# NTHU-LSALAB/KubeShare

Hardware: AMD Instinct MI355X
Metric: aggregate images/sec, co-located shared-GPU pods (higher is better)
Workload: dtype bf16; 1 GPU; model=resnet50, global_batch=512, image_size=224, parallelism=2 pods @ request=0.5, 2/GPU, pods_per_gpu=2, miopen_find=False, lease_accounting=sampled-busy

## Files before the change

kubeshare_amd/models/conv.py:

```python
import torch
import torch.nn as nn


class LowpConv2d(nn.Conv2d):
    _lowp_weight = None

    def _split_input(self, x, w):
        if self.bias is not None or self.padding_mode != "zeros" \
                or isinstance(self.padding, str):
            return None
        if not (w.is_cuda and x.is_cuda and w.dtype == torch.bfloat16
                and x.dim() == 4):
            return None
        from .. import ops
        if not ops.wrw_stream_enabled():
            return None
        if x.dtype != torch.bfloat16:
            if not (x.is_floating_point()
                    and torch.is_autocast_enabled("cuda")
                    and torch.get_autocast_dtype("cuda") == torch.bfloat16):
                return None
            x = x.to(torch.bfloat16)
        return x

    def forward(self, x):
        w = self._lowp_weight
        if w is None:
            return super().forward(x)
        xs = self._split_input(x, w)
        if xs is None:
            return self._conv_forward(x, w, self.bias)
        from .. import ops
        return ops.conv2d_split(xs, w, self.stride, self.padding,
                                self.dilation, self.groups)
```

kubeshare_amd/ops/__init__.py:

```python
from __future__ import annotations

import os

_HERE = os.path.dirname(os.path.abspath(__file__))
_BUILD_DIR = os.path.join(_HERE, "_build")
_SRCS = [os.path.join(_HERE, "hip", "ks_ops.hip"),
         os.path.join(_HERE, "hip", "bn_relu.hip"),
         os.path.join(_HERE, "hip", "pool.hip"),
         os.path.join(_HERE, "hip", "bn_pool.hip"),
         os.path.join(_HERE, "hip", "bn_join.hip"),
         os.path.join(_HERE, "hip", "bias_relu.hip"),
         os.path.join(_HERE, "hip", "cast.hip"),
         os.path.join(_HERE, "hip", "conv_split.hip"),
         os.path.join(_HERE, "hip", "grad_bucket.hip")]

_ext = None


def build_extension(verbose: bool = False):
    import torch
    from torch.utils import cpp_extension

    os.environ.setdefault("PYTORCH_ROCM_ARCH", "gfx950")
    os.makedirs(_BUILD_DIR, exist_ok=True)
# ... 322 lines not shown
                 and x.is_contiguous(memory_format=torch.channels_last))
    if supported and res is not None and res.dtype != torch.bfloat16:
        res = res.to(torch.bfloat16)
    if not supported:
        y = torch.nn.functional.batch_norm(
            x, bn.running_mean, bn.running_var, bn.weight, bn.bias,
            bn.training, bn.momentum, bn.eps)
        if res is not None:
            y = y + res
        y = torch.relu(y) if relu else y
        return (y, y) if fork else y
    if res is not None and not res.is_contiguous(
            memory_format=torch.channels_last):
        res = res.contiguous(memory_format=torch.channels_last)
    fn = _bn_relu_autograd()
    return fn.apply(x, res, bn.weight, bn.bias, bn.running_mean,
                    bn.running_var, bn.training, bn.momentum, bn.eps, relu,
                    fork)


_BNJoinFn = None


def bn_join_enabled() -> bool:
    return os.environ.get("KUBESHARE_BN_JOIN", "1") != "0"


def _bn_join_autograd():
    global _BNJoinFn
    if _BNJoinFn is not None:
        return _BNJoinFn
    import torch

    class BNJoinFn(torch.autograd.Function):

        @staticmethod
        def forward(ctx, x, x_d, weight, bias, running_mean, running_var,
                    momentum, eps, weight_d, bias_d, running_mean_d,
                    running_var_d, momentum_d, eps_d, fork):
            ext = _load()
            w32, b32 = weight.float(), bias.float()
            wd32, bd32 = weight_d.float(), bias_d.float()
            ctx.set_materialize_grads(False)
            ctx.wdtype = weight.dtype
            ctx.wdtype_d = weight_d.dtype
            ctx.legacy_reduce = bn_reduce_legacy()
            ctx.masked = bn_mask_enabled()
            out = ext.bn_join_fwd_train(
                x, w32, b32, running_mean, running_var, momentum, eps,
                x_d, wd32, bd32, running_mean_d, running_var_d, momentum_d,
                eps_d, ctx.masked, ctx.legacy_reduce)
            y = out[0]
            ctx.save_for_backward(x, x_d, out[5] if ctx.masked else y, w32,
                                  wd32, *out[1:5])
            return (y, y.view_as(y)) if fork else y

        @staticmethod
        def backward(ctx, dy, dy2=None):
            x, x_d, ym, w32, wd32, mean, invstd, mean_d, invstd_d = \
                ctx.saved_tensors
            if dy is None:
                dy, dy2 = dy2, None
            if dy is None:
                return (None,) * 15
            dx, dx_d, dscale, dbias, dscale_d = _load().bn_join_bwd(
                x, x_d, ym, dy, dy2, w32, wd32, mean, invstd, mean_d,
                invstd_d, ctx.masked, ctx.legacy_reduce)
            return (dx, dx_d, dscale.to(ctx.wdtype), dbias.to(ctx.wdtype),
                    None, None, None, None, dscale_d.to(ctx.wdtype_d),
                    dbias.clone().to(ctx.wdtype_d), None, None, None, None,
                    None)

    _BNJoinFn = BNJoinFn
    return BNJoinFn


def bn_join_supported(x, x_d) -> bool:
    import torch

    return (x.dim() == 4 and x.shape == x_d.shape
            and x.size(1) % 8 == 0 and x.size(1) <= 2048
            and all(t.is_cuda and t.dtype == torch.bfloat16
                    and t.is_contiguous(memory_format=torch.channels_last)
                    for t in (x, x_d)))


def bn_join(x, bn, x_d, bn_d, fork=False):
    if not (bn_join_enabled() and bn.training and bn_d.training
            and bn_join_supported(x, x_d)):
        return bn_relu(x, bn, res=bn_relu(x_d, bn_d, relu=False), fork=fork)
    fn = _BNJoinFn or _bn_join_autograd()
    return fn.apply(x, x_d, bn.weight, bn.bias, bn.running_mean,
                    bn.running_var, bn.momentum, bn.eps, bn_d.weight,
                    bn_d.bias, bn_d.running_mean, bn_d.running_var,
                    bn_d.momentum, bn_d.eps, fork)


_CastWeightsFn = None


def _cast_weights_autograd():
    global _CastWeightsFn
    if _CastWeightsFn is not None:
        return _CastWeightsFn
    import torch

    class CastWeightsFn(torch.autograd.Function):

        @staticmethod
        def forward(ctx, *weights):
            ctx.set_materialize_grads(False)
            return tuple(_load().cast_f32_to_bf16_multi(list(weights)))

        @staticmethod
        def backward(ctx, *grads):
            wgrad_join()
            out = list(grads)
            idx = [i for i, g in enumerate(grads)
                   if g is not None and g.dtype == torch.bfloat16]
            if idx:
                cast = _load().cast_bf16_to_f32_multi(
                    [grads[i] for i in idx])
                for i, g in zip(idx, cast):
                    out[i] = g
            return tuple(out)

    _CastWeightsFn = CastWeightsFn
    return CastWeightsFn


def cast_weights_bf16(weights):
    fn = _CastWeightsFn or _cast_weights_autograd()
    return fn.apply(*weights)


def lowp_weights_enabled() -> bool:
    return os.environ.get("KUBESHARE_LOWP_WEIGHTS", "1") != "0"


def stage_lowp_weights(convs):
    import torch

    if not convs or not lowp_weights_enabled():
        return []
    if not torch.is_autocast_enabled("cuda") or \
            torch.get_autocast_dtype("cuda") != torch.bfloat16:
        return []
    weights = [m.weight for m in convs]
    if not all(w.is_cuda and w.dtype == torch.float32 for w in weights):
        return []
    wgrad_join()
    for m, w in zip(convs, cast_weights_bf16(weights)):
        m._lowp_weight = w
    return convs


def clear_lowp_weights(convs):
    for m in convs:
        m._lowp_weight = None


def wrw_stream_enabled() -> bool:
    return os.environ.get("KUBESHARE_WRW_STREAM", "1") != "0"


def conv2d_split(x, w, stride=(1, 1), padding=(0, 0), dilation=(1, 1),
                 groups=1):
    def two(v):
        return [int(v), int(v)] if isinstance(v, int) else [int(i) for i in v]
    return _load().conv2d_split(x, w, two(stride), two(padding),
                                two(dilation), int(groups))


def wgrad_join():
    if _ext is not None:
        _ext.wgrad_join()


_POOL_CONFIGS = ((3, 2, 1), (2, 2, 0))
_MaxPoolNHWCFn = None


def _pool_int(v):
    if type(v) is int:
        return v
    if isinstance(v, (tuple, list)) and len(v) == 2 and v[0] == v[1] \
            and type(v[0]) is int:
        return v[0]
    return None


def _pool_cfg(kernel_size, stride, padding):
    if stride is None or stride == () or stride == []:
        stride = kernel_size
    return (_pool_int(kernel_size), _pool_int(stride), _pool_int(padding))


def _pool_cfg_supported(x, cfg) -> bool:
    import torch

    if cfg not in _POOL_CONFIGS or x.dim() != 4:
        return False
    n, c, h, w = x.shape
    k, _, p = cfg
    return (x.is_cuda and x.dtype == torch.bfloat16
            and c % 8 == 0 and 8 <= c <= 2048 and n >= 1
            and h + 2 * p >= k and w + 2 * p >= k
            and n * h * w < 2 ** 31
            and x.is_contiguous(memory_format=torch.channels_last))


def fused_pool_enabled() -> bool:
    return os.environ.get("KUBESHARE_FUSED_POOL", "1") != "0"


def max_pool_supported(x, kernel_size, stride=None, padding=0) -> bool:
    return _pool_cfg_supported(x, _pool_cfg(kernel_size, stride, padding))


def _max_pool_autograd():
    global _MaxPoolNHWCFn
    if _MaxPoolNHWCFn is not None:
        return _MaxPoolNHWCFn
    import torch
    from torch.autograd.function import once_differentiable

    class MaxPoolNHWCFn(torch.autograd.Function):

        @staticmethod
        def forward(ctx, x, k, s, p, want_idx):
            out = _load().max_pool_nhwc_fwd(x, k, s, p, want_idx)
            if want_idx:
                ctx.save_for_backward(out[1])
                ctx.input_sizes = list(x.shape)
                ctx.cfg = (k, s, p)
            return out[0]

        @staticmethod
        @once_differentiable
        def backward(ctx, dy):
            (idx,) = ctx.saved_tensors
            if not dy.is_contiguous(memory_format=torch.channels_last):
                dy = dy.contiguous(memory_format=torch.channels_last)
            k, s, p = ctx.cfg
            dx = _load().max_pool_nhwc_bwd(dy, idx, ctx.input_sizes,
                                           k, s, p)
            return dx, None, None, None, None

    _MaxPoolNHWCFn = MaxPoolNHWCFn
    return MaxPoolNHWCFn


def max_pool_nhwc(x, kernel_size, stride=None, padding=0):
    import torch

    cfg = _pool_cfg(kernel_size, stride, padding)
    if not _pool_cfg_supported(x, cfg):
        return torch.nn.functional.max_pool2d(x, kernel_size, stride,
                                              padding)
    want_idx = torch.is_grad_enabled() and x.requires_grad
    fn = _MaxPoolNHWCFn or _max_pool_autograd()
    return fn.apply(x, *cfg, want_idx)


_BNReLUMaxPoolNHWCFn = None


def bn_pool_enabled() -> bool:
    return os.environ.get("KUBESHARE_BN_POOL", "1") != "0"


def bn_relu_pool_supported(x, kernel_size, stride=None, padding=0) -> bool:
    return _pool_cfg_supported(x, _pool_cfg(kernel_size, stride, padding))


def _bn_relu_pool_autograd():
    global _BNReLUMaxPoolNHWCFn
    if _BNReLUMaxPoolNHWCFn is not None:
        return _BNReLUMaxPoolNHWCFn
    import torch
    from torch.autograd.function import once_differentiable

    class BNReLUMaxPoolNHWCFn(torch.autograd.Function):

        @staticmethod
        def forward(ctx, x, weight, bias, running_mean, running_var,
                    training, momentum, eps, k, s, p, want_idx):
            ext = _load()
            w32 = weight.float()
            b32 = bias.float()
            if not training:
                return ext.bn_relu_pool_fwd_eval(
                    x, w32, b32, running_mean.float(), running_var.float(),
                    eps, k, s, p)[0]
            legacy = bn_reduce_legacy()
            out = ext.bn_relu_pool_fwd_train(
                x, w32, b32, running_mean, running_var, momentum, eps,
                k, s, p, want_idx, legacy)
            if want_idx:
                ctx.save_for_backward(x, out[3], out[1], out[2], w32, b32)
                ctx.cfg = (k, s, p)
                ctx.wdtype = weight.dtype
                ctx.legacy_reduce = legacy
            return out[0]

        @staticmethod
        @once_differentiable
        def backward(ctx, dy):
            x, idx, mean, invstd, w32, b32 = ctx.saved_tensors
            if not dy.is_contiguous(memory_format=torch.channels_last):
                dy = dy.contiguous(memory_format=torch.channels_last)
            dx, dscale, dbias = _load().bn_relu_pool_bwd(
                x, dy, idx, w32, b32, mean, invstd, *ctx.cfg,
                ctx.legacy_reduce)
            return (dx, dscale.to(ctx.wdtype), dbias.to(ctx.wdtype)) + \
                (None,) * 9

    _BNReLUMaxPoolNHWCFn = BNReLUMaxPoolNHWCFn
    return BNReLUMaxPoolNHWCFn


def bn_relu_pool(x, bn, kernel_size, stride=None, padding=0):
    import torch

    cfg = _pool_cfg(kernel_size, stride, padding)
    fused = bn_pool_enabled() and _pool_cfg_supported(x, cfg)
    want_idx = False
    if fused:
        want_idx = torch.is_grad_enabled() and (
            x.requires_grad or bn.weight.requires_grad
            or bn.bias.requires_grad)
        fused = bn.training or not want_idx
    if not fused:
        return max_pool_nhwc(bn_relu(x, bn), kernel_size, stride, padding)
    fn = _BNReLUMaxPoolNHWCFn or _bn_relu_pool_autograd()
    return fn.apply(x, bn.weight, bn.bias, bn.running_mean, bn.running_var,
                    bn.training, bn.momentum, bn.eps, *cfg, want_idx)


_BiasReLUFn = None
_BiasReLUMaxPoolNHWCFn = None


def bias_relu_enabled() -> bool:
    return os.environ.get("KUBESHARE_BIAS_RELU", "1") != "0"


def bias_relu_supported(x) -> bool:
    import torch

    if x.dim() != 4:
        return False
    n, c, h, w = x.shape
    return (x.is_cuda and x.dtype == torch.bfloat16
            and c % 8 == 0 and 8 <= c <= 2048
            and n >= 1 and h >= 1 and w >= 1 and n * h * w < 2 ** 31
            and x.is_contiguous(memory_format=torch.channels_last))


def bias_relu_pool_supported(x, kernel_size, stride=None, padding=0) -> bool:
    return _pool_cfg_supported(x, _pool_cfg(kernel_size, stride, padding))


def _bias_relu_autograd():
    global _BiasReLUFn
    if _BiasReLUFn is not None:
        return _BiasReLUFn
    import torch
    from torch.autograd.function import once_differentiable

    class BiasReLUFn(torch.autograd.Function):

        @staticmethod
        def forward(ctx, x, bias):
            y = _load().bias_relu_fwd(
                x, bias.detach().float().contiguous())
            ctx.save_for_backward(y)
            ctx.bdtype = bias.dtype
            return y

        @staticmethod
        @once_differentiable
        def backward(ctx, dy):
            (y,) = ctx.saved_tensors
            if not dy.is_contiguous(memory_format=torch.channels_last):
                dy = dy.contiguous(memory_format=torch.channels_last)
            dx, db = _load().bias_relu_bwd(dy, y)
            return dx, db.to(ctx.bdtype)

    _BiasReLUFn = BiasReLUFn
    return BiasReLUFn


def _bias_relu_pool_autograd():
    global _BiasReLUMaxPoolNHWCFn
    if _BiasReLUMaxPoolNHWCFn is not None:
        return _BiasReLUMaxPoolNHWCFn
    import torch
    from torch.autograd.function import once_differentiable

    class BiasReLUMaxPoolNHWCFn(torch.autograd.Function):

        @staticmethod
        def forward(ctx, x, bias, k, s, p, want_idx):
            out = _load().bias_relu_pool_fwd(
                x, bias.detach().float().contiguous(), k, s, p, want_idx)
            if want_idx:
                ctx.save_for_backward(out[1], out[0])
                ctx.input_sizes = list(x.shape)
                ctx.cfg = (k, s, p)
                ctx.bdtype = bias.dtype
            return out[0]

        @staticmethod
        @once_differentiable
        def backward(ctx, dy):
            idx, y = ctx.saved_tensors
            if not dy.is_contiguous(memory_format=torch.channels_last):
                dy = dy.contiguous(memory_format=torch.channels_last)
            dx, db = _load().bias_relu_pool_bwd(dy, idx, y, ctx.input_sizes,
                                                *ctx.cfg)
            return dx, db.to(ctx.bdtype), None, None, None, None

    _BiasReLUMaxPoolNHWCFn = BiasReLUMaxPoolNHWCFn
    return BiasReLUMaxPoolNHWCFn


def bias_relu(x, bias):
    import torch

    if not bias_relu_supported(x) or not bias.is_cuda:
        return torch.relu(x + bias.to(x.dtype).view(1, -1, 1, 1))
    fn = _BiasReLUFn or _bias_relu_autograd()
    return fn.apply(x, bias)


def bias_relu_pool(x, bias, kernel_size, stride=None, padding=0):
    import torch

    cfg = _pool_cfg(kernel_size, stride, padding)
    if not _pool_cfg_supported(x, cfg) or not bias.is_cuda:
        if bias_relu_supported(x) and bias.is_cuda:
            return max_pool_nhwc(bias_relu(x, bias), kernel_size, stride,
                                 padding)
        y = torch.relu(x + bias.to(x.dtype).view(1, -1, 1, 1))
        return torch.nn.functional.max_pool2d(y, kernel_size, stride,
                                              padding)
    want_idx = torch.is_grad_enabled() and (x.requires_grad
                                            or bias.requires_grad)
    fn = _BiasReLUMaxPoolNHWCFn or _bias_relu_pool_autograd()
    return fn.apply(x, bias, *cfg, want_idx)


class PendingBNReLU:

    __slots__ = ("x", "bn")

    def __init__(self, x, bn):
        self.x = x
        self.bn = bn

    def materialize(self):
        return bn_relu(self.x, self.bn)


def fuse_model(model):
    _load()
    for m in model.modules():
        if hasattr(m, "fused_ops"):
            m.fused_ops = True
    return model
```

kubeshare_amd/ops/hip/cast.hip:

```cpp
#include <hip/hip_runtime.h>
#include <torch/extension.h>
#include <ATen/cuda/CUDAContext.h>

#include <vector>

#include "cast_common.h"

#define KS_CAST_THREADS 256
#define KS_CAST_VPT 4
#define KS_CAST_CHUNK (KS_CAST_THREADS * KS_CAST_VPT * 8)
#define KS_CAST_MAX_TENSORS 128

typedef __attribute__((ext_vector_type(8))) unsigned short cast_ushort8;

struct CastMultiArgs {
  const void* src[KS_CAST_MAX_TENSORS];
  void* dst[KS_CAST_MAX_TENSORS];
  long long n[KS_CAST_MAX_TENSORS];
  int blk[KS_CAST_MAX_TENSORS + 1];
  int count;
};
static_assert(sizeof(CastMultiArgs) <= 4096,
              "CastMultiArgs must fit the 4 KiB kernel-argument segment");

// ... 18 lines not shown
  CastF8 f;
  f.lo = make_float4(cast_bf16_to_f32(u[0]), cast_bf16_to_f32(u[1]),
                     cast_bf16_to_f32(u[2]), cast_bf16_to_f32(u[3]));
  f.hi = make_float4(cast_bf16_to_f32(u[4]), cast_bf16_to_f32(u[5]),
                     cast_bf16_to_f32(u[6]), cast_bf16_to_f32(u[7]));
  return f;
}

template <bool TO_BF16>
__global__ void __launch_bounds__(KS_CAST_THREADS)
cast_multi_kernel(const CastMultiArgs a) {
  const int b = blockIdx.x;
  int lo = 0, hi = a.count - 1;
  while (lo < hi) {
    int mid = (lo + hi + 1) >> 1;
    if (a.blk[mid] <= b) lo = mid; else hi = mid - 1;
  }
  const long long base = (long long)(b - a.blk[lo]) * KS_CAST_CHUNK;
  const long long rem = a.n[lo] - base;
  const int len = rem < KS_CAST_CHUNK ? (int)rem : KS_CAST_CHUNK;
  const float* __restrict__ f32p;
  const unsigned short* __restrict__ srcb;
  float* __restrict__ dstf;
  unsigned short* __restrict__ bf16p;
  if (TO_BF16) {
    f32p = static_cast<const float*>(a.src[lo]) + base;
    bf16p = static_cast<unsigned short*>(a.dst[lo]) + base;
  } else {
    srcb = static_cast<const unsigned short*>(a.src[lo]) + base;
    dstf = static_cast<float*>(a.dst[lo]) + base;
  }
  const int tid = threadIdx.x;
  const bool vec = TO_BF16
      ? (((uintptr_t)f32p | (uintptr_t)bf16p) & 15) == 0
      : (((uintptr_t)srcb | (uintptr_t)dstf) & 15) == 0;
  if (!vec) {
    for (int k = tid; k < len; k += KS_CAST_THREADS) {
      if (TO_BF16) bf16p[k] = cast_f32_to_bf16(f32p[k]);
      else dstf[k] = cast_bf16_to_f32(srcb[k]);
    }
    return;
  }
  const int len8 = len >> 3;
  if (TO_BF16) {
    const float4* s4 = reinterpret_cast<const float4*>(f32p);
    cast_ushort8* d8 = reinterpret_cast<cast_ushort8*>(bf16p);
    if (len == KS_CAST_CHUNK) {
      CastF8 v[KS_CAST_VPT];
#pragma unroll
      for (int u = 0; u < KS_CAST_VPT; u++) {
        const int k = tid + u * KS_CAST_THREADS;
        v[u].lo = s4[2 * k];
        v[u].hi = s4[2 * k + 1];
      }
#pragma unroll
      for (int u = 0; u < KS_CAST_VPT; u++)
        d8[tid + u * KS_CAST_THREADS] = cast_pack8(v[u]);
      return;
    }
    for (int k = tid; k < len8; k += KS_CAST_THREADS) {
      CastF8 v;
      v.lo = s4[2 * k];
      v.hi = s4[2 * k + 1];
      d8[k] = cast_pack8(v);
    }
    for (int k = len8 * 8 + tid; k < len; k += KS_CAST_THREADS)
      bf16p[k] = cast_f32_to_bf16(f32p[k]);
  } else {
    const cast_ushort8* s8 = reinterpret_cast<const cast_ushort8*>(srcb);
    float4* d4 = reinterpret_cast<float4*>(dstf);
    if (len == KS_CAST_CHUNK) {
      cast_ushort8 v[KS_CAST_VPT];
#pragma unroll
      for (int u = 0; u < KS_CAST_VPT; u++)
        v[u] = s8[tid + u * KS_CAST_THREADS];
#pragma unroll
      for (int u = 0; u < KS_CAST_VPT; u++) {
        const int k = tid + u * KS_CAST_THREADS;
        const CastF8 f = cast_unpack8(v[u]);
        d4[2 * k] = f.lo;
        d4[2 * k + 1] = f.hi;
      }
      return;
    }
    for (int k = tid; k < len8; k += KS_CAST_THREADS) {
      const CastF8 f = cast_unpack8(s8[k]);
      d4[2 * k] = f.lo;
      d4[2 * k + 1] = f.hi;
    }
    for (int k = len8 * 8 + tid; k < len; k += KS_CAST_THREADS)
      dstf[k] = cast_bf16_to_f32(srcb[k]);
  }
}

namespace {

template <bool TO_BF16>
std::vector<c10::optional<torch::Tensor>> cast_multi(
    const std::vector<c10::optional<torch::Tensor>>& src, const char* name) {
  const auto from = TO_BF16 ? at::kFloat : at::kBFloat16;
  const auto to = TO_BF16 ? at::kBFloat16 : at::kFloat;
  auto stream = at::cuda::getCurrentCUDAStream();
  const long long max_blocks = 1LL << 30;
  CastMultiArgs a = {};
  a.count = 0;
  a.blk[0] = 0;
  auto flush = [&]() {
    if (a.count == 0) return;
    hipLaunchKernelGGL(cast_multi_kernel<TO_BF16>, dim3(a.blk[a.count]),
                       dim3(KS_CAST_THREADS), 0, stream.stream(), a);
    a.count = 0;
  };
  std::vector<c10::optional<torch::Tensor>> out(src.size());
  for (size_t t = 0; t < src.size(); t++) {
    if (!src[t].has_value() || !src[t]->defined()) continue;
    const torch::Tensor& s = *src[t];
    TORCH_CHECK(s.is_cuda() && s.scalar_type() == from, name,
                ": CUDA tensors of the source dtype expected");
    if (!s.is_non_overlapping_and_dense() ||
        s.get_device() != stream.device_index()) {
      out[t] = s.to(to);
      continue;
    }
    torch::Tensor d = at::empty_strided(s.sizes(), s.strides(),
                                        s.options().dtype(to));
    out[t] = d;
    const long long n = s.numel();
    if (n == 0) continue;
    const long long nb = (n + KS_CAST_CHUNK - 1) / KS_CAST_CHUNK;
    TORCH_CHECK(nb <= max_blocks, name, ": tensor too large");
    if (a.count == KS_CAST_MAX_TENSORS || a.blk[a.count] + nb > max_blocks)
      flush();
    a.src[a.count] = s.data_ptr();
    a.dst[a.count] = d.data_ptr();
    a.n[a.count] = n;
    a.blk[a.count + 1] = a.blk[a.count] + (int)nb;
    a.count++;
  }
  flush();
  return out;
}

}

std::vector<c10::optional<torch::Tensor>> cast_f32_to_bf16_multi(
    std::vector<c10::optional<torch::Tensor>> src) {
  return cast_multi<true>(src, "cast_f32_to_bf16_multi");
}

std::vector<c10::optional<torch::Tensor>> cast_bf16_to_f32_multi(
    std::vector<c10::optional<torch::Tensor>> src) {
  return cast_multi<false>(src, "cast_bf16_to_f32_multi");
}
```

kubeshare_amd/ops/hip/conv_split.hip:

```cpp
#include <torch/extension.h>
#include <ATen/cuda/CUDAContext.h>
#include <ATen/cuda/CUDAEvent.h>
#include <c10/cuda/CUDAGraphsC10Utils.h>
#include <c10/cuda/CUDAGuard.h>
#include <c10/cuda/CUDAStream.h>

#include <cstdlib>
#include <memory>
#include <mutex>
#include <vector>

namespace {

struct WgradSide {
  c10::optional<c10::cuda::CUDAStream> stream;
  std::unique_ptr<at::cuda::CUDAEvent> fork, done;
  bool pending = false;
};

std::mutex g_mu;
std::vector<WgradSide> g_side;

int side_priority() {
  const char* v = std::getenv("KUBESHARE_WRW_PRIORITY");
  return v && v[0] ? std::atoi(v) : 0;
}

WgradSide& side_for(c10::DeviceIndex dev) {
  if (g_side.size() <= (size_t)dev) g_side.resize((size_t)dev + 1);
  WgradSide& s = g_side[dev];
  if (!s.stream.has_value()) {
    s.stream = c10::cuda::getStreamFromPool(side_priority(), dev);
    s.fork = std::make_unique<at::cuda::CUDAEvent>();
    s.done = std::make_unique<at::cuda::CUDAEvent>();
  }
  return s;
}

bool capturing() {
  return c10::cuda::currentStreamCaptureStatusMayInitCtx() !=
         c10::cuda::CaptureStatus::None;
}

}

struct Conv2dSplitFn : public torch::autograd::Function<Conv2dSplitFn> {
  static torch::Tensor forward(torch::autograd::AutogradContext* ctx,
                               torch::Tensor x, torch::Tensor w,
                               std::vector<int64_t> stride,
                               std::vector<int64_t> padding,
                               std::vector<int64_t> dilation, int64_t groups) {
    TORCH_CHECK(x.is_cuda() && w.is_cuda() && x.dim() == 4 && w.dim() == 4,
                "conv2d_split: 4-d CUDA tensors expected");
    TORCH_CHECK(x.get_device() == w.get_device(),
                "conv2d_split: x and w on different devices");
    TORCH_CHECK(stride.size() == 2 && padding.size() == 2 &&
                    dilation.size() == 2,
                "conv2d_split: stride, padding and dilation take two ints");
    ctx->save_for_backward({x, w});
    ctx->saved_data["stride"] = stride;
    ctx->saved_data["padding"] = padding;
    ctx->saved_data["dilation"] = dilation;
    ctx->saved_data["groups"] = groups;
    return at::convolution(x, w, c10::nullopt, stride, padding, dilation,
                           false, {0, 0},
                           groups);
  }

  static torch::autograd::variable_list backward(
      torch::autograd::AutogradContext* ctx,
      torch::autograd::variable_list grads) {
    TORCH_CHECK(!at::GradMode::is_enabled(),
                "conv2d_split: double backward (create_graph=True) is not "
                "supported; set KUBESHARE_WRW_STREAM=0 for the stock "
                "convolution");
    const auto saved = ctx->get_saved_variables();
    const torch::Tensor& x = saved[0];
    const torch::Tensor& w = saved[1];
    const torch::Tensor& dy = grads[0];
    const auto stride = ctx->saved_data["stride"].toIntVector();
    const auto padding = ctx->saved_data["padding"].toIntVector();
    const auto dilation = ctx->saved_data["dilation"].toIntVector();
    const int64_t groups = ctx->saved_data["groups"].toInt();
    torch::Tensor dx, dw;
    const torch::autograd::variable_list none(6);
    if (!dy.defined()) return none;
    const bool need_dx = ctx->needs_input_grad(0);
    const bool need_dw = ctx->needs_input_grad(1);
    auto half = [&](bool data) {
      auto out = at::convolution_backward(
          dy, x, w, c10::nullopt, stride, padding, dilation,
          false, {0, 0}, groups,
          {data, !data, false});
      return data ? std::get<0>(out) : std::get<1>(out);
    };
    const c10::DeviceIndex dev = (c10::DeviceIndex)dy.get_device();
    c10::cuda::CUDAGuard device_guard(dev);
    if (!need_dw || capturing()) {
      if (need_dx) dx = half(true);
      if (need_dw) dw = half(false);
      return {dx, dw, none[2], none[3], none[4], none[5]};
    }
    const auto cur = c10::cuda::getCurrentCUDAStream(dev);
    std::lock_guard<std::mutex> lock(g_mu);
    WgradSide& s = side_for(dev);
    const c10::cuda::CUDAStream side = *s.stream;
    s.fork->record(cur);
    s.fork->block(side);
    if (need_dx) dx = half(true);
    dy.record_stream(side);
    x.record_stream(side);
    {
      c10::cuda::CUDAStreamGuard stream_guard(side);
      dw = half(false);
    }
    dw.record_stream(cur);
    s.done->record(side);
    s.pending = true;
    return {dx, dw, none[2], none[3], none[4], none[5]};
  }
};

torch::Tensor conv2d_split(torch::Tensor x, torch::Tensor w,
                           std::vector<int64_t> stride,
                           std::vector<int64_t> padding,
                           std::vector<int64_t> dilation, int64_t groups) {
  return Conv2dSplitFn::apply(x, w, stride, padding, dilation, groups);
}

void wgrad_join() {
  std::lock_guard<std::mutex> lock(g_mu);
  for (size_t d = 0; d < g_side.size(); d++) {
    WgradSide& s = g_side[d];
    if (!s.pending) continue;
    c10::cuda::CUDAGuard device_guard((c10::DeviceIndex)d);
    if (capturing()) continue;
    s.done->block(c10::cuda::getCurrentCUDAStream((c10::DeviceIndex)d));
    s.pending = false;
  }
}

bool wgrad_pending() {
  std::lock_guard<std::mutex> lock(g_mu);
  for (const WgradSide& s : g_side)
    if (s.pending) return true;
  return false;
}
```

kubeshare_amd/ops/hip/ks_ops.hip:

```cpp
#include <hip/hip_runtime.h>
#include <torch/extension.h>
#include <ATen/cuda/CUDAContext.h>

#include <type_traits>
#include <vector>

#define WAVE 64

__global__ void burn_kernel(long long ticks, float* sink) {
  long long start = wall_clock64();
  float acc = threadIdx.x * 1e-9f;
  while (wall_clock64() - start < ticks) {
#pragma unroll
    for (int i = 0; i < 64; i++) acc = fmaf(acc, 1.0000001f, 1e-12f);
  }
  if (acc == 12345.678f) sink[0] = acc;
}

void burn(double ms, int64_t blocks, int64_t threads) {
  long long ticks = (long long)(ms * 100000.0);
  auto stream = at::cuda::getCurrentCUDAStream();
  static float* sink = nullptr;
  if (!sink) {
    if (hipMalloc(&sink, sizeof(float)) != hipSuccess)
// ... 161 lines not shown
  auto stream = at::cuda::getCurrentCUDAStream();
  for (size_t t = 0; t < params.size(); t++) {
    auto& p = params[t];
    auto& g = grads[t];
    auto& v = momenta[t];
    TORCH_CHECK(p.is_cuda() && p.scalar_type() == at::kFloat &&
                    p.is_non_overlapping_and_dense() &&
                    g.sizes() == p.sizes() && g.strides() == p.strides() &&
                    v.strides() == p.strides() &&
                    g.scalar_type() == at::kFloat &&
                    v.scalar_type() == at::kFloat,
                "sgd_momentum_: f32 dense tensors with matching strides "
                "(any memory format: the update is elementwise over the "
                "flat storage)");
    long long n = p.numel();
    int threads = 256;
    int blocks = (int)std::min<long long>(2048, (n / 4 + threads - 1) / threads + 1);
    hipLaunchKernelGGL(sgd_mom_f32_kernel, dim3(blocks), dim3(threads), 0,
                       stream.stream(), p.data_ptr<float>(),
                       g.data_ptr<float>(), v.data_ptr<float>(), (float)lr,
                       (float)mu, (float)wd, n);
  }
}

template <typename G>
static int64_t sgd_momentum_multi_impl(
    const std::vector<torch::Tensor>& params,
    const std::vector<c10::optional<torch::Tensor>>& grads,
    const std::vector<torch::Tensor>& momenta, double lr, double mu,
    double wd) {
  constexpr bool g_f32 = std::is_same<G, float>::value;
  const auto gtype = g_f32 ? at::kFloat : at::kBFloat16;
  TORCH_CHECK(params.size() == grads.size() &&
                  params.size() == momenta.size(),
              "sgd_momentum_multi_: params, grads and momenta differ in "
              "length");
  auto stream = at::cuda::getCurrentCUDAStream();
  const long long max_blocks = 1LL << 30;
  SgdMultiArgs<G> a = {};
  a.lr = (float)lr;
  a.mu = (float)mu;
  a.wd = (float)wd;
  a.count = 0;
  a.blk[0] = 0;
  int64_t launches = 0;
  std::vector<torch::Tensor> keep;
  auto flush = [&]() {
    if (a.count == 0) return;
    hipLaunchKernelGGL(sgd_mom_multi_f32_kernel<G>, dim3(a.blk[a.count]),
                       dim3(KS_SGD_THREADS), 0, stream.stream(), a);
    launches++;
    a.count = 0;
  };
  for (size_t t = 0; t < params.size(); t++) {
    if (!grads[t].has_value() || !grads[t]->defined()) continue;
    auto& p = params[t];
    auto& v = momenta[t];
    torch::Tensor g = *grads[t];
    TORCH_CHECK(g.sizes() == p.sizes() && g.is_cuda() &&
                    g.scalar_type() == gtype,
                "sgd_momentum_multi_: ", g_f32 ? "f32" : "bf16",
                " CUDA gradient of the parameter's shape expected");
    if (g_f32 && g.strides() != p.strides()) {
      g = at::empty_like(p).copy_(g);
      keep.push_back(g);
    }
    TORCH_CHECK(p.is_cuda() && p.scalar_type() == at::kFloat &&
                    p.is_non_overlapping_and_dense() &&
                    g.sizes() == p.sizes() && g.strides() == p.strides() &&
                    v.strides() == p.strides() &&
                    g.scalar_type() == gtype &&
                    v.scalar_type() == at::kFloat,
                "sgd_momentum_: f32 dense tensors with matching strides "
                "(any memory format: the update is elementwise over the "
                "flat storage)");
    TORCH_CHECK(v.is_cuda() && v.sizes() == p.sizes() &&
                    p.get_device() == stream.device_index() &&
                    g.get_device() == p.get_device() &&
                    v.get_device() == p.get_device(),
                "sgd_momentum_multi_: parameter, gradient and momentum "
                "must live on the current device and share a shape");
    const long long n = p.numel();
    if (n == 0) continue;
    const long long nb = (n + KS_SGD_CHUNK - 1) / KS_SGD_CHUNK;
    TORCH_CHECK(nb <= max_blocks, "sgd_momentum_multi_: tensor too large");
    if (a.count == KS_SGD_MAX_TENSORS || a.blk[a.count] + nb > max_blocks)
      flush();
    a.p[a.count] = p.data_ptr<float>();
    a.g[a.count] = static_cast<const G*>(g.data_ptr());
    a.v[a.count] = v.data_ptr<float>();
    a.n[a.count] = n;
    a.blk[a.count + 1] = a.blk[a.count] + (int)nb;
    a.count++;
  }
  flush();
  return launches;
}

int64_t sgd_momentum_multi_(std::vector<torch::Tensor> params,
                            std::vector<c10::optional<torch::Tensor>> grads,
                            std::vector<torch::Tensor> momenta, double lr,
                            double mu, double wd) {
  return sgd_momentum_multi_impl<float>(params, grads, momenta, lr, mu, wd);
}

int64_t sgd_momentum_multi_bf16g_(
    std::vector<torch::Tensor> params,
    std::vector<c10::optional<torch::Tensor>> grads,
    std::vector<torch::Tensor> momenta, double lr, double mu, double wd) {
  return sgd_momentum_multi_impl<unsigned short>(params, grads, momenta, lr,
                                                 mu, wd);
}

std::vector<torch::Tensor> bn_relu_fwd_train(
    torch::Tensor x, torch::Tensor weight, torch::Tensor bias,
    torch::Tensor running_mean, torch::Tensor running_var, double momentum,
    double eps, c10::optional<torch::Tensor> res, bool relu,
    bool legacy_reduce, bool want_mask);
torch::Tensor bn_relu_fwd_eval(torch::Tensor x, torch::Tensor weight,
                               torch::Tensor bias, torch::Tensor rmean,
                               torch::Tensor rvar, double eps,
                               c10::optional<torch::Tensor> res, bool relu);
std::vector<torch::Tensor> bn_relu_bwd(
    torch::Tensor x, c10::optional<torch::Tensor> y, torch::Tensor dy,
    torch::Tensor weight, torch::Tensor bias, torch::Tensor mean,
    torch::Tensor invstd, bool need_dres, bool relu,
    c10::optional<torch::Tensor> dy2, bool legacy_reduce,
    c10::optional<torch::Tensor> mask);

std::vector<torch::Tensor> bn_join_fwd_train(
    torch::Tensor x, torch::Tensor weight, torch::Tensor bias,
    torch::Tensor running_mean, torch::Tensor running_var, double momentum,
    double eps, torch::Tensor x_d, torch::Tensor weight_d,
    torch::Tensor bias_d, torch::Tensor running_mean_d,
    torch::Tensor running_var_d, double momentum_d, double eps_d,
    bool want_mask, bool legacy_reduce);
std::vector<torch::Tensor> bn_join_bwd(
    torch::Tensor x, torch::Tensor x_d, torch::Tensor y_or_mask,
    torch::Tensor dy, c10::optional<torch::Tensor> dy2, torch::Tensor weight,
    torch::Tensor weight_d, torch::Tensor mean, torch::Tensor invstd,
    torch::Tensor mean_d, torch::Tensor invstd_d, bool use_mask,
    bool legacy_reduce);

int64_t grad_pack_multi(std::vector<c10::optional<torch::Tensor>> srcs,
                        torch::Tensor flat, std::vector<int64_t> offsets,
                        double scale, std::vector<torch::Tensor> like);
int64_t grad_unpack_multi(torch::Tensor flat, std::vector<int64_t> offsets,
                          std::vector<c10::optional<torch::Tensor>> dsts);

std::vector<c10::optional<torch::Tensor>> cast_f32_to_bf16_multi(
    std::vector<c10::optional<torch::Tensor>> src);
std::vector<c10::optional<torch::Tensor>> cast_bf16_to_f32_multi(
    std::vector<c10::optional<torch::Tensor>> src);

std::vector<torch::Tensor> max_pool_nhwc_fwd(torch::Tensor x, int64_t k,
                                             int64_t s, int64_t p,
                                             bool want_idx);
torch::Tensor max_pool_nhwc_bwd(torch::Tensor dy, torch::Tensor idx,
                                std::vector<int64_t> input_sizes, int64_t k,
                                int64_t s, int64_t p);

std::vector<torch::Tensor> bn_relu_pool_fwd_train(
    torch::Tensor x, torch::Tensor weight, torch::Tensor bias,
    torch::Tensor running_mean, torch::Tensor running_var, double momentum,
    double eps, int64_t k, int64_t s, int64_t p, bool want_idx,
    bool legacy_reduce);
std::vector<torch::Tensor> bn_relu_pool_fwd_eval(
    torch::Tensor x, torch::Tensor weight, torch::Tensor bias,
    torch::Tensor rmean, torch::Tensor rvar, double eps, int64_t k,
    int64_t s, int64_t p);
std::vector<torch::Tensor> bn_relu_pool_bwd(
    torch::Tensor x, torch::Tensor dy, torch::Tensor idx,
    torch::Tensor weight, torch::Tensor bias, torch::Tensor mean,
    torch::Tensor invstd, int64_t k, int64_t s, int64_t p,
    bool legacy_reduce);

torch::Tensor bias_relu_fwd(torch::Tensor x, torch::Tensor bias);
std::vector<torch::Tensor> bias_relu_bwd(torch::Tensor dy, torch::Tensor y);
std::vector<torch::Tensor> bias_relu_pool_fwd(torch::Tensor x,
                                              torch::Tensor bias, int64_t k,
                                              int64_t s, int64_t p,
                                              bool want_idx);
std::vector<torch::Tensor> bias_relu_pool_bwd(
    torch::Tensor dy, torch::Tensor idx, torch::Tensor y,
    std::vector<int64_t> input_sizes, int64_t k, int64_t s, int64_t p);

torch::Tensor conv2d_split(torch::Tensor x, torch::Tensor w,
                           std::vector<int64_t> stride,
                           std::vector<int64_t> padding,
                           std::vector<int64_t> dilation, int64_t groups);
void wgrad_join();
bool wgrad_pending();

PYBIND11_MODULE(TORCH_EXTENSION_NAME, m) {
  m.def("burn", &burn, "occupy the GPU for ~ms milliseconds",
        py::arg("ms"), py::arg("blocks") = 1024, py::arg("threads") = 256);
  m.def("sgd_momentum_", &sgd_momentum_,
        "fused SGD+momentum update (in-place)");
  m.def("sgd_momentum_multi_", &sgd_momentum_multi_,
        "fused SGD+momentum update of all tensors in as few launches as "
        "the kernel-argument limit allows; a None gradient skips its "
        "tensor; returns the number of launches");
  m.def("sgd_momentum_multi_bf16g_", &sgd_momentum_multi_bf16g_,
        "sgd_momentum_multi_ reading bf16 gradients that have the "
        "parameters' sizes and strides");
  m.def("grad_pack_multi", &grad_pack_multi, py::arg("srcs"),
        py::arg("flat"), py::arg("offsets"), py::arg("scale"),
        py::arg("like"),
        "flat[offsets[t] + i] = (f32(scale) * srcs[t][i]).to(flat.dtype) "
        "over the storage of like[t]'s layout; None writes zeros; returns "
        "the number of launches");
  m.def("grad_unpack_multi", &grad_unpack_multi, py::arg("flat"),
        py::arg("offsets"), py::arg("dsts"),
        "dsts[t][i] = float(flat[offsets[t] + i]) over dsts[t]'s dense "
        "storage; None is skipped; returns the number of launches");
  m.def("bn_relu_fwd_train", &bn_relu_fwd_train, py::arg("x"),
        py::arg("weight"), py::arg("bias"), py::arg("running_mean"),
        py::arg("running_var"), py::arg("momentum"), py::arg("eps"),
        py::arg("res"), py::arg("relu"), py::arg("legacy_reduce") = false,
        py::arg("want_mask") = false,
        "{y, mean, invstd} and, with want_mask (res and relu only), the "
        "uint8 (N, H, W, C/8) ReLU mask");
  m.def("bn_relu_fwd_eval", &bn_relu_fwd_eval);
  m.def("bn_relu_bwd", &bn_relu_bwd, py::arg("x"), py::arg("y"),
        py::arg("dy"), py::arg("weight"), py::arg("bias"), py::arg("mean"),
        py::arg("invstd"), py::arg("need_dres"), py::arg("relu"),
        py::arg("dy2") = py::none(), py::arg("legacy_reduce") = false,
        py::arg("mask") = py::none(),
        "{dx, dscale, dbias[, dres]}; with mask (residual BNs) y may be "
        "None");
  m.def("bn_join_fwd_train", &bn_join_fwd_train, py::arg("x"),
        py::arg("weight"), py::arg("bias"), py::arg("running_mean"),
        py::arg("running_var"), py::arg("momentum"), py::arg("eps"),
        py::arg("x_d"), py::arg("weight_d"), py::arg("bias_d"),
        py::arg("running_mean_d"), py::arg("running_var_d"),
        py::arg("momentum_d"), py::arg("eps_d"), py::arg("want_mask"),
        py::arg("legacy_reduce") = false,
        "relu(bn(x) + bn_d(x_d)): {y, mean, invstd, mean_d, invstd_d} and, "
        "with want_mask, the uint8 (N, H, W, C/8) ReLU mask");
  m.def("bn_join_bwd", &bn_join_bwd, py::arg("x"), py::arg("x_d"),
        py::arg("y_or_mask"), py::arg("dy"), py::arg("dy2"),
        py::arg("weight"), py::arg("weight_d"), py::arg("mean"),
        py::arg("invstd"), py::arg("mean_d"), py::arg("invstd_d"),
        py::arg("use_mask"), py::arg("legacy_reduce") = false,
        "{dx, dx_d, dscale, dbias, dscale_d}; dbias serves both BNs");
  m.def("cast_f32_to_bf16_multi", &cast_f32_to_bf16_multi,
        "f32 -> bf16 (torch rounding) of every tensor of a list in as few "
        "launches as the kernel-argument limit allows; None stays None");
  m.def("cast_bf16_to_f32_multi", &cast_bf16_to_f32_multi,
        "bf16 -> f32 of every tensor of a list; None stays None");
  m.def("max_pool_nhwc_fwd", &max_pool_nhwc_fwd);
  m.def("max_pool_nhwc_bwd", &max_pool_nhwc_bwd);
  m.def("bn_relu_pool_fwd_train", &bn_relu_pool_fwd_train, py::arg("x"),
        py::arg("weight"), py::arg("bias"), py::arg("running_mean"),
        py::arg("running_var"), py::arg("momentum"), py::arg("eps"),
        py::arg("k"), py::arg("s"), py::arg("p"), py::arg("want_idx"),
        py::arg("legacy_reduce") = false,
        "{y, mean, invstd} and, with want_idx, the one-byte window codes");
  m.def("bn_relu_pool_fwd_eval", &bn_relu_pool_fwd_eval,
        "{y} from the running statistics; no codes");
  m.def("bn_relu_pool_bwd", &bn_relu_pool_bwd, py::arg("x"), py::arg("dy"),
        py::arg("idx"), py::arg("weight"), py::arg("bias"), py::arg("mean"),
        py::arg("invstd"), py::arg("k"), py::arg("s"), py::arg("p"),
        py::arg("legacy_reduce") = false, "{dx, dscale, dbias}");
  m.def("bias_relu_fwd", &bias_relu_fwd, py::arg("x"), py::arg("bias"),
        "y = bf16(relu(f32(x) + bias)), bias f32");
  m.def("bias_relu_bwd", &bias_relu_bwd, py::arg("dy"), py::arg("y"),
        "{dx, db}");
  m.def("bias_relu_pool_fwd", &bias_relu_pool_fwd, py::arg("x"),
        py::arg("bias"), py::arg("k"), py::arg("s"), py::arg("p"),
        py::arg("want_idx"),
        "{y} and, with want_idx, the one-byte window codes");
  m.def("bias_relu_pool_bwd", &bias_relu_pool_bwd, py::arg("dy"),
        py::arg("idx"), py::arg("y"), py::arg("input_sizes"), py::arg("k"),
        py::arg("s"), py::arg("p"), "{dx, db}");
  m.def("conv2d_split", &conv2d_split, py::arg("x"), py::arg("w"),
        py::arg("stride"), py::arg("padding"), py::arg("dilation"),
        py::arg("groups"),
        "bias-free at::convolution; its backward runs the weight gradient "
        "on a side stream (join with wgrad_join)");
  m.def("wgrad_join", &wgrad_join,
        "the current stream waits for every pending side-stream weight "
        "gradient; a no-op with nothing pending");
  m.def("wgrad_pending", &wgrad_pending,
        "True while a side-stream weight gradient has not been joined");
}
```

Measured before the change: 9733 images/s.

## Compute conv data gradients as forward convolutions with mirrored bf16 weights

```diff
diff --git a/kubeshare_amd/models/conv.py b/kubeshare_amd/models/conv.py
--- a/kubeshare_amd/models/conv.py
+++ b/kubeshare_amd/models/conv.py
@@ -4,6 +4,8 @@
 
 class LowpConv2d(nn.Conv2d):
     _lowp_weight = None
+    _dgrad_fwd = False
+    _lowp_mirror = None
 
     def _split_input(self, x, w):
         if self.bias is not None or self.padding_mode != "zeros" \
@@ -32,4 +34,5 @@
             return self._conv_forward(x, w, self.bias)
         from .. import ops
         return ops.conv2d_split(xs, w, self.stride, self.padding,
-                                self.dilation, self.groups)
+                                self.dilation, self.groups,
+                                self._lowp_mirror)
diff --git a/kubeshare_amd/ops/__init__.py b/kubeshare_amd/ops/__init__.py
--- a/kubeshare_amd/ops/__init__.py
+++ b/kubeshare_amd/ops/__init__.py
@@ -498,12 +498,74 @@
     wgrad_join()
     for m, w in zip(convs, cast_weights_bf16(weights)):
         m._lowp_weight = w
+    if torch.is_grad_enabled() and dgrad_fwd_active():
+        flagged = [m for m in convs if getattr(m, "_dgrad_fwd", False)
+                   and m.weight.requires_grad]
+        if flagged:
+            mirrors = _load().mirror_weights_multi(
+                [m._lowp_weight.detach() for m in flagged])
+            for m, wm in zip(flagged, mirrors):
+                m._lowp_mirror = wm
     return convs
 
 
 def clear_lowp_weights(convs):
     for m in convs:
         m._lowp_weight = None
+        m._lowp_mirror = None
+
+
+_DGRAD_FWD_MODES = ("0", "1x1", "3x3", "all", "")
+
+
+def dgrad_fwd_mode() -> str:
+    v = os.environ.get("KUBESHARE_DGRAD_FWD", "")
+    if v not in _DGRAD_FWD_MODES:
+        raise ValueError(f"KUBESHARE_DGRAD_FWD={v!r}: one of 0, 1x1, 3x3, "
+                         "all expected")
+    return v
+
+
+def dgrad_fwd_active() -> bool:
+    import torch
+
+    mode = dgrad_fwd_mode()
+    if mode == "0":
+        return False
+    return mode != "" or not torch.backends.cudnn.deterministic
+
+
+def _dgrad_fwd_signature(m):
+    import torch.nn as nn
+
+    if not isinstance(m, nn.Conv2d) or m.bias is not None \
+            or m.padding_mode != "zeros" or isinstance(m.padding, str):
+        return None
+    k = m.kernel_size[0]
+    if tuple(m.kernel_size) != (k, k) or k not in (1, 3) \
+            or tuple(m.stride) != (1, 1) or tuple(m.dilation) != (1, 1) \
+            or m.groups != 1 or tuple(m.padding) != (k // 2, k // 2):
+        return None
+    return (m.in_channels, m.out_channels, k)
+
+
+def dgrad_fwd_flags(model, mode=None):
+    from ..models.conv import LowpConv2d
+
+    mode = dgrad_fwd_mode() if mode is None else mode
+    sigs = {m: _dgrad_fwd_signature(m) for m in model.modules()}
+    present = {s for s in sigs.values() if s is not None}
+    flags = {}
+    for m, sig in sigs.items():
+        if not isinstance(m, LowpConv2d):
+            continue
+        ok = sig is not None and mode != "0"
+        if ok and mode in ("1x1", "3x3"):
+            ok = mode == f"{sig[2]}x{sig[2]}"
+        if ok and mode != "all":
+            ok = (sig[1], sig[0], sig[2]) in present
+        flags[m] = ok
+    return flags
 
 
 def wrw_stream_enabled() -> bool:
@@ -511,11 +573,15 @@
 
 
 def conv2d_split(x, w, stride=(1, 1), padding=(0, 0), dilation=(1, 1),
-                 groups=1):
+                 groups=1, mirror=None):
     def two(v):
         return [int(v), int(v)] if isinstance(v, int) else [int(i) for i in v]
     return _load().conv2d_split(x, w, two(stride), two(padding),
-                                two(dilation), int(groups))
+                                two(dilation), int(groups), mirror)
+
+
+def mirror_weights(weights):
+    return _load().mirror_weights_multi(list(weights))
 
 
 def wgrad_join():
@@ -815,4 +881,8 @@
     for m in model.modules():
         if hasattr(m, "fused_ops"):
             m.fused_ops = True
+    from ..models.resnet import ResNet
+    if isinstance(model, ResNet):
+        for m, flag in dgrad_fwd_flags(model).items():
+            m._dgrad_fwd = flag
     return model
diff --git a/kubeshare_amd/ops/hip/cast.hip b/kubeshare_amd/ops/hip/cast.hip
--- a/kubeshare_amd/ops/hip/cast.hip
+++ b/kubeshare_amd/ops/hip/cast.hip
@@ -194,3 +194,142 @@
     std::vector<c10::optional<torch::Tensor>> src) {
   return cast_multi<false>(src, "cast_bf16_to_f32_multi");
 }
+
+#define KS_MIRROR_THREADS 256
+#define KS_MIRROR_TILE 64
+#define KS_MIRROR_LD (KS_MIRROR_TILE + 2)
+#define KS_MIRROR_MAX_TENSORS ((4096 - 8) / 32)
+
+struct MirrorMultiArgs {
+  const void* src[KS_MIRROR_MAX_TENSORS];
+  void* dst[KS_MIRROR_MAX_TENSORS];
+  int K[KS_MIRROR_MAX_TENSORS];
+  int C[KS_MIRROR_MAX_TENSORS];
+  int RS[KS_MIRROR_MAX_TENSORS];
+  int blk[KS_MIRROR_MAX_TENSORS + 1];
+  int count;
+};
+static_assert(sizeof(MirrorMultiArgs) <= 4096,
+              "MirrorMultiArgs must fit the 4 KiB kernel-argument segment");
+static_assert(KS_MIRROR_THREADS == 4 * KS_MIRROR_TILE &&
+                  KS_MIRROR_TILE % 8 == 0,
+              "a block covers the tile in two passes of 32 rows, eight "
+              "8-element vectors per row");
+
+__global__ void __launch_bounds__(KS_MIRROR_THREADS)
+mirror_multi_kernel(const MirrorMultiArgs a) {
+  __shared__ unsigned short tile[KS_MIRROR_TILE][KS_MIRROR_LD];
+  const int b = blockIdx.x;
+  int lo = 0, hi = a.count - 1;
+  while (lo < hi) {
+    int mid = (lo + hi + 1) >> 1;
+    if (a.blk[mid] <= b) lo = mid; else hi = mid - 1;
+  }
+  const int K = a.K[lo], C = a.C[lo], RS = a.RS[lo];
+  const int tiles_c = (C + KS_MIRROR_TILE - 1) / KS_MIRROR_TILE;
+  const int tiles_k = (K + KS_MIRROR_TILE - 1) / KS_MIRROR_TILE;
+  int lb = b - a.blk[lo];
+  const int c0 = (lb % tiles_c) * KS_MIRROR_TILE;
+  lb /= tiles_c;
+  const int k0 = (lb % tiles_k) * KS_MIRROR_TILE;
+  const int tap = lb / tiles_k;
+  const long long srow = (long long)RS * C, drow = (long long)RS * K;
+  const unsigned short* __restrict__ src =
+      static_cast<const unsigned short*>(a.src[lo]) +
+      (long long)(RS - 1 - tap) * C;
+  unsigned short* __restrict__ dst =
+      static_cast<unsigned short*>(a.dst[lo]) + (long long)tap * K;
+  const int row = threadIdx.x >> 3;
+  const int v = (threadIdx.x & 7) * 8;
+  const bool vin = (C & 7) == 0 && ((uintptr_t)a.src[lo] & 15) == 0;
+  const bool vout = (K & 7) == 0 && ((uintptr_t)a.dst[lo] & 15) == 0;
+#pragma unroll
+  for (int p = 0; p < 2; p++) {
+    const int k = row + p * 32;
+    const int gk = k0 + k, gc = c0 + v;
+    if (gk >= K) continue;
+    const unsigned short* s = src + gk * srow + gc;
+    if (vin) {
+      if (gc < C) {
+        const cast_ushort8 x = *reinterpret_cast<const cast_ushort8*>(s);
+#pragma unroll
+        for (int j = 0; j < 8; j++) tile[k][v + j] = x[j];
+      }
+    } else {
+      for (int j = 0; j < 8; j++)
+        if (gc + j < C) tile[k][v + j] = s[j];
+    }
+  }
+  __syncthreads();
+#pragma unroll
+  for (int p = 0; p < 2; p++) {
+    const int c = row + p * 32;
+    const int gc = c0 + c, gk = k0 + v;
+    if (gc >= C) continue;
+    unsigned short* d = dst + gc * drow + gk;
+    if (vout) {
+      if (gk < K) {
+        cast_ushort8 o;
+#pragma unroll
+        for (int j = 0; j < 8; j++) o[j] = tile[v + j][c];
+        *reinterpret_cast<cast_ushort8*>(d) = o;
+      }
+    } else {
+      for (int j = 0; j < 8; j++)
+        if (gk + j < K) d[j] = tile[v + j][c];
+    }
+  }
+}
+
+static torch::Tensor mirror_weight_eager(const torch::Tensor& w) {
+  return w.flip({2, 3}).transpose(0, 1).contiguous(
+      at::MemoryFormat::ChannelsLast);
+}
+
+std::vector<torch::Tensor> mirror_weights_multi(
+    std::vector<torch::Tensor> src) {
+  auto stream = at::cuda::getCurrentCUDAStream();
+  const long long max_blocks = 1LL << 30;
+  MirrorMultiArgs a = {};
+  a.count = 0;
+  a.blk[0] = 0;
+  auto flush = [&]() {
+    if (a.count == 0) return;
+    hipLaunchKernelGGL(mirror_multi_kernel, dim3(a.blk[a.count]),
+                       dim3(KS_MIRROR_THREADS), 0, stream.stream(), a);
+    a.count = 0;
+  };
+  std::vector<torch::Tensor> out(src.size());
+  for (size_t t = 0; t < src.size(); t++) {
+    const torch::Tensor& s = src[t];
+    TORCH_CHECK(s.defined() && s.dim() == 4,
+                "mirror_weights_multi: 4-d weights (K,C,R,S) expected");
+    if (!s.is_cuda() || s.scalar_type() != at::kBFloat16 ||
+        s.get_device() != stream.device_index() ||
+        !s.is_contiguous(at::MemoryFormat::ChannelsLast)) {
+      out[t] = mirror_weight_eager(s);
+      continue;
+    }
+    const long long K = s.size(0), C = s.size(1), RS = s.size(2) * s.size(3);
+    torch::Tensor d = at::empty(
+        {C, K, s.size(2), s.size(3)},
+        s.options().memory_format(at::MemoryFormat::ChannelsLast));
+    out[t] = d;
+    if (s.numel() == 0) continue;
+    const long long nb = RS * ((K + KS_MIRROR_TILE - 1) / KS_MIRROR_TILE) *
+                         ((C + KS_MIRROR_TILE - 1) / KS_MIRROR_TILE);
+    TORCH_CHECK(s.numel() < (1LL << 31) && nb <= max_blocks,
+                "mirror_weights_multi: tensor too large");
+    if (a.count == KS_MIRROR_MAX_TENSORS || a.blk[a.count] + nb > max_blocks)
+      flush();
+    a.src[a.count] = s.data_ptr();
+    a.dst[a.count] = d.data_ptr();
+    a.K[a.count] = (int)K;
+    a.C[a.count] = (int)C;
+    a.RS[a.count] = (int)RS;
+    a.blk[a.count + 1] = a.blk[a.count] + (int)nb;
+    a.count++;
+  }
+  flush();
+  return out;
+}
diff --git a/kubeshare_amd/ops/hip/conv_split.hip b/kubeshare_amd/ops/hip/conv_split.hip
--- a/kubeshare_amd/ops/hip/conv_split.hip
+++ b/kubeshare_amd/ops/hip/conv_split.hip
@@ -49,7 +49,8 @@
                                torch::Tensor x, torch::Tensor w,
                                std::vector<int64_t> stride,
                                std::vector<int64_t> padding,
-                               std::vector<int64_t> dilation, int64_t groups) {
+                               std::vector<int64_t> dilation, int64_t groups,
+                               c10::optional<torch::Tensor> mirror) {
     TORCH_CHECK(x.is_cuda() && w.is_cuda() && x.dim() == 4 && w.dim() == 4,
                 "conv2d_split: 4-d CUDA tensors expected");
     TORCH_CHECK(x.get_device() == w.get_device(),
@@ -57,7 +58,34 @@
     TORCH_CHECK(stride.size() == 2 && padding.size() == 2 &&
                     dilation.size() == 2,
                 "conv2d_split: stride, padding and dilation take two ints");
-    ctx->save_for_backward({x, w});
+    const bool routed = mirror.has_value() && mirror->defined();
+    if (routed) {
+      const int64_t r = w.size(2);
+      TORCH_CHECK(stride[0] == 1 && stride[1] == 1 && dilation[0] == 1 &&
+                      dilation[1] == 1 && groups == 1,
+                  "conv2d_split: a mirrored weight needs stride 1, "
+                  "dilation 1 and groups 1");
+      TORCH_CHECK(w.size(3) == r && (r == 1 || r == 3) &&
+                      padding[0] == (r - 1) / 2 && padding[1] == (r - 1) / 2,
+                  "conv2d_split: a mirrored weight needs a 1x1 or 3x3 "
+                  "kernel with \"same\" padding");
+      TORCH_CHECK(x.scalar_type() == at::kBFloat16 &&
+                      w.scalar_type() == at::kBFloat16 &&
+                      mirror->scalar_type() == at::kBFloat16,
+                  "conv2d_split: a mirrored weight needs bf16 x, w and "
+                  "mirror");
+      TORCH_CHECK(mirror->is_cuda() &&
+                      mirror->get_device() == x.get_device() &&
+                      mirror->dim() == 4 && mirror->size(0) == w.size(1) &&
+                      mirror->size(1) == w.size(0) &&
+                      mirror->size(2) == r && mirror->size(3) == r,
+                  "conv2d_split: the mirrored weight of a (K,C,R,S) weight "
+                  "is (C,K,R,S) on x's device");
+      ctx->save_for_backward({x, w, *mirror});
+    } else {
+      ctx->save_for_backward({x, w});
+    }
+    ctx->saved_data["routed"] = routed;
     ctx->saved_data["stride"] = stride;
     ctx->saved_data["padding"] = padding;
     ctx->saved_data["dilation"] = dilation;
@@ -83,7 +111,7 @@
     const auto dilation = ctx->saved_data["dilation"].toIntVector();
     const int64_t groups = ctx->saved_data["groups"].toInt();
     torch::Tensor dx, dw;
-    const torch::autograd::variable_list none(6);
+    const torch::autograd::variable_list none(7);
     if (!dy.defined()) return none;
     const bool need_dx = ctx->needs_input_grad(0);
     const bool need_dw = ctx->needs_input_grad(1);
@@ -94,12 +122,26 @@
           {data, !data, false});
       return data ? std::get<0>(out) : std::get<1>(out);
     };
+    const bool routed = ctx->saved_data["routed"].toBool();
+    auto data_half = [&]() {
+      if (!routed) return half(true);
+      const torch::Tensor& wm = saved[2];
+      const int64_t ph = wm.size(2) - 1 - padding[0];
+      const int64_t pw = wm.size(3) - 1 - padding[1];
+      const torch::Tensor g =
+          dy.is_contiguous(at::MemoryFormat::ChannelsLast)
+              ? dy
+              : dy.contiguous(at::MemoryFormat::ChannelsLast);
+      return at::convolution(g, wm, c10::nullopt, {1, 1}, {ph, pw}, {1, 1},
+                             false, {0, 0},
+                             1);
+    };
     const c10::DeviceIndex dev = (c10::DeviceIndex)dy.get_device();
     c10::cuda::CUDAGuard device_guard(dev);
     if (!need_dw || capturing()) {
-      if (need_dx) dx = half(true);
+      if (need_dx) dx = data_half();
       if (need_dw) dw = half(false);
-      return {dx, dw, none[2], none[3], none[4], none[5]};
+      return {dx, dw, none[2], none[3], none[4], none[5], none[6]};
     }
     const auto cur = c10::cuda::getCurrentCUDAStream(dev);
     std::lock_guard<std::mutex> lock(g_mu);
@@ -107,7 +149,7 @@
     const c10::cuda::CUDAStream side = *s.stream;
     s.fork->record(cur);
     s.fork->block(side);
-    if (need_dx) dx = half(true);
+    if (need_dx) dx = data_half();
     dy.record_stream(side);
     x.record_stream(side);
     {
@@ -117,15 +159,17 @@
     dw.record_stream(cur);
     s.done->record(side);
     s.pending = true;
-    return {dx, dw, none[2], none[3], none[4], none[5]};
+    return {dx, dw, none[2], none[3], none[4], none[5], none[6]};
   }
 };
 
 torch::Tensor conv2d_split(torch::Tensor x, torch::Tensor w,
                            std::vector<int64_t> stride,
                            std::vector<int64_t> padding,
-                           std::vector<int64_t> dilation, int64_t groups) {
-  return Conv2dSplitFn::apply(x, w, stride, padding, dilation, groups);
+                           std::vector<int64_t> dilation, int64_t groups,
+                           c10::optional<torch::Tensor> mirror) {
+  return Conv2dSplitFn::apply(x, w, stride, padding, dilation, groups,
+                              mirror);
 }
 
 void wgrad_join() {
diff --git a/kubeshare_amd/ops/hip/ks_ops.hip b/kubeshare_amd/ops/hip/ks_ops.hip
--- a/kubeshare_amd/ops/hip/ks_ops.hip
+++ b/kubeshare_amd/ops/hip/ks_ops.hip
@@ -337,6 +337,8 @@
     std::vector<c10::optional<torch::Tensor>> src);
 std::vector<c10::optional<torch::Tensor>> cast_bf16_to_f32_multi(
     std::vector<c10::optional<torch::Tensor>> src);
+std::vector<torch::Tensor> mirror_weights_multi(
+    std::vector<torch::Tensor> src);
 
 std::vector<torch::Tensor> max_pool_nhwc_fwd(torch::Tensor x, int64_t k,
                                              int64_t s, int64_t p,
@@ -373,7 +375,8 @@
 torch::Tensor conv2d_split(torch::Tensor x, torch::Tensor w,
                            std::vector<int64_t> stride,
                            std::vector<int64_t> padding,
-                           std::vector<int64_t> dilation, int64_t groups);
+                           std::vector<int64_t> dilation, int64_t groups,
+                           c10::optional<torch::Tensor> mirror);
 void wgrad_join();
 bool wgrad_pending();
 
@@ -434,6 +437,9 @@
         "launches as the kernel-argument limit allows; None stays None");
   m.def("cast_bf16_to_f32_multi", &cast_bf16_to_f32_multi,
         "bf16 -> f32 of every tensor of a list; None stays None");
+  m.def("mirror_weights_multi", &mirror_weights_multi,
+        "bf16 (K,C,R,S) weights -> new channels-last (C,K,R,S) tensors "
+        "with out[c,k,r,s] = in[k,c,R-1-r,S-1-s], one launch per list");
   m.def("max_pool_nhwc_fwd", &max_pool_nhwc_fwd);
   m.def("max_pool_nhwc_bwd", &max_pool_nhwc_bwd);
   m.def("bn_relu_pool_fwd_train", &bn_relu_pool_fwd_train, py::arg("x"),
@@ -461,9 +467,10 @@
         py::arg("s"), py::arg("p"), "{dx, db}");
   m.def("conv2d_split", &conv2d_split, py::arg("x"), py::arg("w"),
         py::arg("stride"), py::arg("padding"), py::arg("dilation"),
-        py::arg("groups"),
+        py::arg("groups"), py::arg("mirror") = py::none(),
         "bias-free at::convolution; its backward runs the weight gradient "
-        "on a side stream (join with wgrad_join)");
+        "on a side stream (join with wgrad_join) and, given the mirrored "
+        "weight, the data gradient as a forward convolution");
   m.def("wgrad_join", &wgrad_join,
         "the current stream waits for every pending side-stream weight "
         "gradient; a no-op with nothing pending");
```

Result: faster. 10140 images/s (median of 6 runs) (+4.1%).
